# chao1224/MoleculeSDE

Hardware: AMD Instinct MI355X
Metric: molecules/sec pretrain step (SchNet+SDE VE, bs256) (higher is better)
Workload: dtype f32; 1 GPU; PCQM4Mv2-shaped pretrain step: GIN5x300 + SchNet(6x128f,51g,rc10) + EBM_node_dot_prod contrastive + SDEModel2Dto3D_02 VE; fwd+bwd+Adam; molecules_per_gpu=256, global_batch=256, parallelism=dp1

## Files before the change

### include/msde_hip.h

```cpp
#ifndef MSDE_HIP_H
#define MSDE_HIP_H

#ifdef __cplusplus
extern "C" {
#endif

#define MSDE_EINVAL (-1)
#define MSDE_EUNSUP (-2)

int msde_abi_version(void);
const char* msde_target_arch(void);

int msde_radius_count(const float* pos, const int* batch, const int* mol_ptr, int N, float r2,
                      int max_nbr, int* deg, void* stream);
int msde_exclusive_scan_i32(const int* in, int* out, int n, void* stream);
int msde_radius_fill(const float* pos, const int* batch, const int* mol_ptr, int N, float r2,
                     int max_nbr, const int* rowptr, int* src, int* dst, float* dist, int E_cap,
                     void* stream);


int msde_plan_build(const int* x_raw, int K, const int* atom_off, const int* bond_src, const int* bond_dst,
                    const int* bond_attr, const int* bond_off, const int* mol_atoms, const int* mol_bonds,
                    int B, int N_cap, int Eb_cap, int Ee_cap, int P_cap, int Er_cap, int max_nbr, int* mol_ptr,
                    int* bond_ptr, int* pair_ptr, int* sizes, int* batch_i32, int* atom_codes, int* z_codes, int* b_rowptr,
// ... 419 lines not shown
                              const unsigned long long* group_seed, const int* group_ptr, int G, int n, int max_group_atoms,
                              float snr, float scale_eps, float* x, float* x_mean, void* stream);
int msde_pc_predictor_grouped(const float* out, const float* pos, const float* noise, const float* par, const long long* step,
                              const unsigned long long* group_seed, const int* group_ptr, int G, int n, float* x, float* x_mean,
                              int* group_bad, void* stream);
int msde_l1_energy_force_loss(const float* E, const float* y, int B, const float* dE, const float* f, int n3, float fsign, float ce,
                              float cf, float* loss, float* gE, float* gdE, void* stream);
int msde_randperm(int n, int count, unsigned long long seed, const unsigned long long* seed_dev, int* out,
                  const int* rows_dev, void* stream);
int msde_ve_perturb(const float* pos, const float* noise, const long long* draws, const int* batch, int N,
                    int B, int T, float eps, float sigma_min, float sigma_max, float* pos_out,
                    float* std_out, void* stream);
int msde_ve_perturb_rng(const float* pos, const int* batch, int N, int B, int T, float eps, float sigma_min,
                        float sigma_max, unsigned long long seed, const unsigned long long* seed_dev,
                        float* noise_out, float* pos_out, float* std_out, void* stream);
int msde_ve_pos_loss_fwd(const float* scores, const float* noise, const float* std, float anneal_power,
                         const int* mol_ptr, int N, int B, float* mol_ws, float* loss, void* stream);
int msde_ve_pos_loss_bwd(const float* scores, const float* noise, const float* std, float anneal_power,
                         const int* mol_ptr, const int* batch, int N, int B, const float* g_loss,
                         float* g_scores, void* stream);

int msde_gat_tail_blocks(int N);
int msde_gat_tail_fwd(const float* x, const float* res, const float* ln1_g, const float* ln1_b,
                      const float* W0, const float* b0, const float* W3, const float* b3,
                      const float* ln2_g, const float* ln2_b, int N, int D, float eps1, float eps2,
                      float p_drop, unsigned long long seed, const unsigned long long* seed_dev,
                      int silu_out, float* out, float* y1, float* h0, float* x2, void* stream);
int msde_gat_tail_bwd(const float* g_out, const float* x, const float* y1, const float* h0,
                      const float* x2, const float* ln1_g, const float* W0, const float* W3,
                      const float* ln2_g, const float* ln2_b, int N, int D, float eps1, float eps2,
                      float p_drop, unsigned long long seed, const unsigned long long* seed_dev,
                      int silu_out, float* g_x, float* g_res, float* g_x2, float* a, float* g_h0,
                      float* ln_part, const int* rows_dev, void* stream);

long long msde_escore_mol_saved_floats(int N);
int msde_escore_mol_fwd(const void* const* params, const float* x0, const float* edge_attr, int ld_ea,
                        const float* basis, const int* mol_ptr, int B, const int* rowptr, const int* src,
                        const int* dst, int N, int E, int hidden, int heads, int hidden_coff, int n_max, float p_att,
                        float p_ffn, unsigned long long seed0, const unsigned long long* seed_dev, float eps1,
                        float eps2, float* out, float* saved, void* stream);

long long msde_escore_mol_score_scratch_floats(int E);
int msde_escore_mol_score(const void* const* params, const float* x0, const float* pos, const float* edge_2D, int ld_e2d,
                          int has_dist, const int* mol_ptr, int B, const int* rowptr, const int* src, const int* dst, int N, int E,
                          int hidden, int heads, int hidden_coff, int n_max, float eps1, float eps2, float* scratch, float* out,
                          void* stream);

long long msde_escore_mol_slab_floats(void);
int msde_escore_mol_bwd(const void* const* params, const float* x0, const float* edge_attr, int ld_ea,
                        const float* basis, const int* mol_ptr, int B, const int* rowptr, const int* src,
                        const int* dst, const int* rowptr_s, const int* perm_s, int N, int E, int hidden, int heads,
                        int hidden_coff, int n_max, float p_att, float p_ffn, unsigned long long seed0,
                        const unsigned long long* seed_dev, float eps1, float eps2, const float* saved,
                        const float* g_out, float* g_x0, float* g_edge_attr, int ld_gea, float* slabs, void* stream);

int msde_molnet_head_fwd(const float* h, int ldh, int M, int D, const int* mol_ptr, int B, const int* row_bound,
                         const float* W, const float* bias, int T, float* pool, float* logits, void* stream);
int msde_molnet_bce(const float* logits, const float* y, int B, int T, double* loss_mat, double* stats, float* dlogits,
                    void* stream);
int msde_molnet_head_bwd(const float* dlogits, int B, int T, const float* W, int D, const int* mol_ptr,
                         const int* row_bound, int M, float* dh, int ldh, void* stream);

int msde_qm9_head_train(const float* out, int ldo, int B, int D, const float* W, const float* b, const float* y, int ldy,
                        float mean, float std, int mode, float* pred, float* loss, float* dout, float* dW, float* db,
                        double* loss_acc, void* stream);
int msde_qm9_head_eval(const float* out, int ldo, int B, int D, const float* W, const float* b, const float* y, int ldy,
// ... 26 lines not shown
```

### moleculesde_amd/_lib.py

```python
import ctypes
import os

_HERE = os.path.dirname(os.path.abspath(__file__))
LIB_PATH = os.path.join(_HERE, "csrc", "libmsde_hip.so")

P = ctypes.c_void_p
I = ctypes.c_int
F = ctypes.c_float
LL = ctypes.c_longlong
ULL = ctypes.c_ulonglong

SIGNATURES = {
    "msde_abi_version": [],
    "msde_target_arch": [],
    "msde_radius_count": [P, P, P, I, F, I, P, P],
    "msde_exclusive_scan_i32": [P, P, I, P],
    "msde_radius_fill": [P, P, P, I, F, I, P, P, P, P, I, P],
    "msde_segment_sum_rows": [P, I, P, P, I, I, F, P, I, P],
    "msde_segment_sum_rows2": [P, I, P, P, P, P, I, I, F, P, I, P],
    "msde_pair_gather_add": [P, P, I, P, P, I, I, P, P],
    "msde_pair_gather_add_stats": [P, P, I, P, P, I, I, P, P, P, P],
    "msde_segment_sum_rows_bn": [P, P, I, P, P, I, I, P, P, P, P, I, P],
    "msde_pair_strip": [],
    "msde_pair_bn_dgrad_stats": [P, I, P, P, P, P, P, I, I, I, P, P, P, P],
# ... 119 lines not shown
    "msde_res_layernorm_bwd": [P, P, P, P, P, I, I, P, P, P, P, P],
    "msde_bn_fwd": [P, I, I, P, P, F, F, P, P, I, P, P, P, P, P, P],
    "msde_bn_bwd": [P, P, P, P, P, P, I, I, I, P, P, P, P, P, P],
    "msde_adam_flat": [P, P, P, P, LL, P, P, P, I, F, F, F, F, F, P],
    "msde_ssp_fwd": [P, LL, P, P],
    "msde_ssp_bwd": [P, P, LL, P, P],
    "msde_silu_dropout_fwd": [P, LL, F, ULL, P, P, P],
    "msde_silu_dropout_bwd": [P, P, LL, F, ULL, P, P, P],
    "msde_dropout_rows_fwd": [P, I, I, P, F, ULL, I, P, P, P],
    "msde_dropout_rows_bwd": [P, I, I, P, F, ULL, I, P, P, P],
    "msde_molnet_head_fwd": [P, I, I, I, P, I, P, P, P, I, P, P, P],
    "msde_molnet_bce": [P, P, I, I, P, P, P, P],
    "msde_molnet_head_bwd": [P, I, I, P, I, P, P, I, P, I, P],
    "msde_qm9_head_train": [P, I, I, I, P, P, P, I, F, F, I, P, P, P, P, P, P, P],
    "msde_qm9_head_eval": [P, I, I, I, P, P, P, I, F, F, P, P, P],
    "msde_mul_add_fwd": [P, P, P, LL, P, P],
    "msde_mul_add_bwd": [P, P, P, LL, P, P, P],
    "msde_pc_corrector": [P, P, P, P, P, ULL, I, F, F, P, P, P],
    "msde_pc_predictor": [P, P, P, P, P, ULL, I, P, P, P],
    "msde_pc_corrector_grouped": [P, P, P, P, P, P, P, I, I, I, F, F, P, P, P],
    "msde_pc_predictor_grouped": [P, P, P, P, P, P, P, I, I, P, P, P, P],
    "msde_l1_energy_force_loss": [P, P, I, P, P, I, F, F, F, P, P, P, P],
    "msde_l1_energy_force_loss_acc": [P, P, I, P, P, I, F, F, F, P, P, P, P, P],
    "msde_md17_eval_accumulate": [P, P, I, P, P, I, P, P],
    "msde_md17_gather_batch": [P, P, P, I, I, P, P, I, I, P, P, P, P],
    "msde_randperm": [I, I, ULL, P, P, P, P],
    "msde_ve_perturb": [P, P, P, P, I, I, I, F, F, F, P, P, P],
    "msde_ve_perturb_rng": [P, P, I, I, I, F, F, F, ULL, P, P, P, P, P],
    "msde_ve_pos_loss_fwd": [P, P, P, F, P, I, I, P, P, P],
    "msde_ve_pos_loss_bwd": [P, P, P, F, P, P, I, I, P, P, P],
    "msde_gat_tail_blocks": [I],
    "msde_gat_tail_fwd": [P, P, P, P, P, P, P, P, P, P, I, I, F, F, F, ULL, P, I, P, P, P, P, P],
    "msde_gat_tail_bwd": [P, P, P, P, P, P, P, P, P, P, I, I, F, F, F, ULL, P, I, P, P, P, P, P, P, P, P],
    "msde_escore_mol_saved_floats": [I],
    "msde_escore_mol_fwd": [P, P, P, I, P, P, I, P, P, P, I, I, I, I, I, I, F, F, ULL, P, F, F, P, P, P],
    "msde_escore_mol_score": [P, P, P, P, I, I, P, I, P, P, P, I, I, I, I, I, I, F, F, P, P, P],
    "msde_escore_mol_score_scratch_floats": [I],
    "msde_escore_mol_slab_floats": [],
    "msde_escore_mol_bwd": [P, P, P, I, P, P, I, P, P, P, P, P, I, I, I, I, I, I, F, F, ULL, P, F, F, P, P, P, P, I, P, P],
    "msde_chunk_elems": [],
    "msde_gather_chunks": [P, I, P, P],
    "msde_adam_chunks": [P, P, I, P, P, P, P, P, I, F, F, F, F, F, P],
}


class GemmDesc(ctypes.Structure):
    _fields_ = [("A", P), ("A2", P), ("B", P), ("B2", P), ("bias", P), ("bias2", P), ("C", P), ("Z", P), ("R", P),
                ("rowscale", P),
                ("a_gs", LL), ("b_gs", LL), ("bias_gs", LL), ("c_gs", LL), ("r_gs", LL), ("b_kblk_stride", LL),
                ("M", I), ("N", I), ("K1", I), ("K2", I),
                ("lda", I), ("lda2", I), ("ldb", I), ("ldb2", I), ("ldc", I), ("ldz", I), ("ldr", I),
                ("act", I), ("act_lo", I), ("act_hi", I), ("epi", I), ("flags", I), ("groups", I),
                ("b_kblk_log2", I), ("alpha", F)]


class RsDesc(ctypes.Structure):
    _fields_ = [("A", P), ("A2", P), ("B", P), ("bias", P), ("C", P), ("Z", P), ("R", P), ("Res", P), ("A_out", P),
                ("xf0", P), ("xf1", P), ("xf2", P), ("xf3", P), ("xf4", P), ("stats", P), ("stats_z", P),
                ("stats_mean", P), ("m_valid", P),
                ("M", I), ("N", I), ("K", I),
                ("lda", I), ("lda2", I), ("ldb", I), ("ldc", I), ("ldz", I), ("ldr", I), ("ldres", I), ("lda_out", I),
                ("ld_sz", I),
                ("act", I), ("epi", I), ("flags", I), ("axf", I), ("stats_mode", I), ("rt", I), ("splits", I)]


RS_AXF_NONE, RS_AXF_AFFINE, RS_AXF_BNBWD, RS_AXF_RELU, RS_VEC_STORE = 0, 1, 2, 4, 8
# ... 64 lines not shown
```

### moleculesde_amd/build.py

```python
import os
import subprocess
import sys
from concurrent.futures import ThreadPoolExecutor

HERE = os.path.dirname(os.path.abspath(__file__))
CSRC = os.path.join(HERE, "csrc")
OBJ = os.path.join(CSRC, "build")
LIB = os.path.join(CSRC, "libmsde_hip.so")
SOURCES = ["graph.hip", "gin.hip", "schnet.hip", "cfconv_fused.hip", "cfconv_fused_bwd.hip", "cfconv_pair.hip",
           "sde2d3d.hip", "linear.hip", "gemm_ex.hip", "gemm_rs.hip", "gemm_t2.hip", "gemm_t2_a1.hip", "gemm_t2_a2.hip", "dense_head.hip", "dense_pc.hip", "plan.hip", "dd.hip", "norm.hip",
           "contrastive.hip", "contrastive_infonce.hip", "optim.hip", "pointwise.hip", "gat_tail.hip", "escore_mol.hip", "escore_mol_bwd.hip",
           "molnet_head.hip", "qm9_head.hip", "md17.hip"]
HEADERS = [os.path.join(CSRC, "msde_common.h"), os.path.join(CSRC, "gemm_rs.h"), os.path.join(CSRC, "gemm_rs_epi.h"), os.path.join(CSRC, "gemm_t2.h"), os.path.join(CSRC, "escore_mol.h"),
           os.path.join(HERE, "..", "include", "msde_hip.h")]


def _flags():
    return ["--offload-arch=gfx950", "-O3", "-std=c++17", "-fPIC", "-Wno-unused-result", "-Wno-unused-value"] + \
        os.environ.get("MSDE_HIPCC_FLAGS", "").split()


def _stale(target, deps):
    if not os.path.exists(target):
        return True
    t = os.path.getmtime(target)
    return any(os.path.exists(d) and os.path.getmtime(d) > t for d in deps)


def needs_build():
    srcs = [os.path.join(CSRC, s) for s in SOURCES if os.path.exists(os.path.join(CSRC, s))]
    return _stale(LIB, srcs + HEADERS)


def build(force=False, verbose=True):
    if not force and not needs_build():
        return LIB
    hipcc = os.environ.get("HIPCC", "/opt/rocm/bin/hipcc")
    os.makedirs(OBJ, exist_ok=True)
    flags = _flags()
    stamp = os.path.join(OBJ, "flags.txt")
    old = open(stamp).read() if os.path.exists(stamp) else None
    if old != " ".join(flags):
        force = True
    jobs, objs = [], []
    for s in SOURCES:
        src = os.path.join(CSRC, s)
# ... 25 lines not shown
```

### moleculesde_amd/csrc/gat_tail.hip

```cpp
#include "msde_common.h"

#define GT_THREADS 256
#ifndef GT_LPR
#define GT_LPR 8
#endif
#define GT_ROWS (GT_THREADS / GT_LPR)

__device__ __forceinline__ float gt_sigmoid(float x) {
  float e = expf(-fabsf(x));
  float r = 1.f / (1.f + e);
  return x >= 0.f ? r : e * r;
}

template <int C>
__device__ __forceinline__ float gt_row_sum(float s) {
  s += __shfl_xor(s, 1);
  s += __shfl_xor(s, 2);
  if (GT_LPR >= 8) s += __shfl_xor(s, 4);
  if (GT_LPR >= 16) s += __shfl_xor(s, 8);
  return s;
}
template <int C>
__device__ __forceinline__ void gt_layernorm(const float (&v)[C], float eps, float& mu, float& rs) {
  constexpr float invD = 1.f / (float)(C * GT_LPR);
  float s = 0.f;
#pragma unroll
  for (int k = 0; k < C; ++k) s += v[k];
  mu = gt_row_sum<C>(s) * invD;
  float q = 0.f;
#pragma unroll
  for (int k = 0; k < C; ++k) q = fmaf(v[k] - mu, v[k] - mu, q);
  rs = rsqrtf(gt_row_sum<C>(q) * invD + eps);
}
// ... 171 lines not shown
    float m = 1.f;
    if (p_drop > 0.f) m = msde_uniform(seed, (unsigned long long)(off + j)) >= p_drop ? scale : 0.f;
    t2[j] = a * m;
    u[j] = u[j] * m * da;
  }
  if (live) { gt_store<C>(a_o, off, t2); gt_store<C>(g_h0_o, off, u); }
  gt_gather<C>(u, full);
  gt_matvec_t<C>(W0s, q, full, g);
  if (live) gt_store<C>(g_res, off, g);
  gt_load<C>(x, off, u);
  gt_layernorm<C>(u, eps1, mu, rs);
  c1 = 0.f; c2 = 0.f;
#pragma unroll
  for (int k = 0; k < C; ++k) {
    u[k] = (u[k] - mu) * rs;
    red[rowl][2 * D + q * C + k] = lv * g[k] * u[k];
    red[rowl][3 * D + q * C + k] = lv * g[k];
    float gg = g[k] * prm[q * C + k];
    c1 += gg; c2 = fmaf(gg, u[k], c2);
  }
  c1 = gt_row_sum<C>(c1) * (1.f / D); c2 = gt_row_sum<C>(c2) * (1.f / D);
#pragma unroll
  for (int k = 0; k < C; ++k) t2[k] = rs * (g[k] * prm[q * C + k] - c1 - u[k] * c2);
  if (live) gt_store<C>(g_x, off, t2);
  __syncthreads();
  for (int t = threadIdx.x; t < 4 * D; t += GT_THREADS) {
    float acc = 0.f;
#pragma unroll 8
    for (int r = 0; r < GT_ROWS; ++r) acc += red[r][t];
    ln_part[(size_t)blockIdx.x * 4 * D + t] = acc;
  }
}

extern "C" int msde_gat_tail_blocks(int N) { return (N + GT_ROWS - 1) / GT_ROWS; }

extern "C" int msde_gat_tail_fwd(const float* x, const float* res, const float* ln1_g, const float* ln1_b, const float* W0,
                                 const float* b0, const float* W3, const float* b3, const float* ln2_g,
                                 const float* ln2_b, int N, int D, float eps1, float eps2, float p_drop,
                                 unsigned long long seed, const unsigned long long* seed_dev, int silu_out, float* out,
                                 float* y1, float* h0, float* x2, void* stream) {
  if (N < 0 || !x || !res || !ln1_g || !ln1_b || !W0 || !b0 || !W3 || !b3 || !ln2_g || !ln2_b || !out || !y1 || !h0 || !x2)
    return MSDE_EINVAL;
  if (p_drop < 0.f || p_drop >= 1.f) return MSDE_EINVAL;
  if (D != 32) return MSDE_EUNSUP;
  if (N == 0) return 0;
  MSDE_LAUNCH(gat_tail_fwd_kernel<32>, dim3(msde_gat_tail_blocks(N)), dim3(GT_THREADS), 0, as_stream(stream), x, res, ln1_g,
              ln1_b, W0, b0, W3, b3, ln2_g, ln2_b, N, eps1, eps2, p_drop, seed, seed_dev, silu_out, out, y1, h0, x2);
  MSDE_CHECK_LAUNCH();
  return 0;
}

extern "C" int msde_gat_tail_bwd(const float* g_out, const float* x, const float* y1, const float* h0, const float* x2,
                                 const float* ln1_g, const float* W0, const float* W3, const float* ln2_g,
                                 const float* ln2_b, int N, int D, float eps1, float eps2, float p_drop,
                                 unsigned long long seed, const unsigned long long* seed_dev, int silu_out, float* g_x,
                                 float* g_res, float* g_x2, float* a, float* g_h0, float* ln_part, const int* rows_dev,
                                 void* stream) {
  if (N < 0 || !g_out || !x || !y1 || !h0 || !x2 || !ln1_g || !W0 || !W3 || !ln2_g || !ln2_b || !g_x || !g_res || !g_x2 ||
      !a || !g_h0 || !ln_part)
    return MSDE_EINVAL;
  if (p_drop < 0.f || p_drop >= 1.f) return MSDE_EINVAL;
  if (D != 32) return MSDE_EUNSUP;
  if (N == 0) return 0;
  MSDE_LAUNCH(gat_tail_bwd_kernel<32>, dim3(msde_gat_tail_blocks(N)), dim3(GT_THREADS), 0, as_stream(stream), g_out, x, y1,
              h0, x2, ln1_g, W0, W3, ln2_g, ln2_b, N, rows_dev, eps1, eps2, p_drop, seed, seed_dev, silu_out, g_x, g_res, g_x2,
              a, g_h0,
              ln_part);
  MSDE_CHECK_LAUNCH();
  return 0;
}
```

### moleculesde_amd/csrc/graph.hip

```cpp
#include "msde_common.h"

__global__ void radius_count_kernel(const float* __restrict__ pos, const int* __restrict__ batch,
                                    const int* __restrict__ mol_ptr, int N, float r2, int max_nbr,
                                    int* __restrict__ deg) {
  int i = blockIdx.x * blockDim.x + threadIdx.x;
  if (i >= N) return;
  int m = batch[i];
  int j0 = mol_ptr[m], j1 = mol_ptr[m + 1];
  float xi = pos[3 * i], yi = pos[3 * i + 1], zi = pos[3 * i + 2];
  int cnt = 0;
  for (int j = j0; j < j1 && cnt < max_nbr; ++j) {
    if (j == i) continue;
    float dx = xi - pos[3 * j], dy = yi - pos[3 * j + 1], dz = zi - pos[3 * j + 2];
    float d2 = dx * dx + dy * dy + dz * dz;
    cnt += (d2 < r2) ? 1 : 0;
  }
  deg[i] = cnt;
}

__global__ void radius_fill_kernel(const float* __restrict__ pos, const int* __restrict__ batch,
                                   const int* __restrict__ mol_ptr, int N, float r2, int max_nbr,
                                   const int* __restrict__ rowptr, int* __restrict__ src,
                                   int* __restrict__ dst, float* __restrict__ dist, int E_cap) {
  int i = blockIdx.x * blockDim.x + threadIdx.x;
  if (i < N) {
    int m = batch[i];
    int j0 = mol_ptr[m], j1 = mol_ptr[m + 1];
    float xi = pos[3 * i], yi = pos[3 * i + 1], zi = pos[3 * i + 2];
    int slot = rowptr[i];
    int cnt = 0;
    for (int j = j0; j < j1 && cnt < max_nbr; ++j) {
      if (j == i) continue;
      float dx = xi - pos[3 * j], dy = yi - pos[3 * j + 1], dz = zi - pos[3 * j + 2];
// ... 195 lines not shown
  if (mean != 0.f) scale = 1.f / (float)max(s1 - s0, 1);
  const T* R = reinterpret_cast<const T*>(rows);
  T* O = reinterpret_cast<T*>(out);
  for (int c = lane; c < cols; c += tpr) {
    T acc = vzero<V>();
    int s = s0 + el;
    for (; s + 3 * epl < s1; s += 4 * epl) {
      int e0 = perm ? perm[s] : s, e1 = perm ? perm[s + epl] : s + epl;
      int e2 = perm ? perm[s + 2 * epl] : s + 2 * epl, e3 = perm ? perm[s + 3 * epl] : s + 3 * epl;
      T v0 = R[(size_t)e0 * ldi_cols + c], v1 = R[(size_t)e1 * ldi_cols + c];
      T v2 = R[(size_t)e2 * ldi_cols + c], v3 = R[(size_t)e3 * ldi_cols + c];
      acc = vadd(vadd(vadd(vadd(acc, v0), v1), v2), v3);
    }
    for (; s < s1; s += epl) {
      int e = perm ? perm[s] : s;
      acc = vadd(acc, R[(size_t)e * ldi_cols + c]);
    }
    if (rowptr2 != nullptr && live) {
      const int q1 = rowptr2[i + 1];
      for (int q = rowptr2[i] + el; q < q1; q += epl) {
        int e = perm2 ? perm2[q] : q;
        acc = vadd(acc, R[(size_t)e * ldi_cols + c]);
      }
    }
    for (int o = tpr; o < group; o <<= 1) {
      float* a = reinterpret_cast<float*>(&acc);
#pragma unroll
      for (int k = 0; k < V; ++k) a[k] += __shfl_xor(a[k], o);
    }
    if (live && el == 0) O[(size_t)i * ldo_cols + c] = vscale(acc, scale);
  }
}

static inline int seg_epl(int N, int tpr) {
  const int force = 0;
  if (force) return force * tpr <= 64 ? force : 1;
  const int wide = 0;
  if (tpr >= 32 && !wide) return 1;
  int epl = 1;
  while (epl < 4 && tpr * epl * 2 <= 64 && (long)N * tpr * epl < 256L * 1024) epl *= 2;
  return epl;
}

extern "C" int msde_segment_sum_rows2(const float* rows, int ldi, const int* rowptr, const int* perm, const int* rowptr2,
                                      const int* perm2, int N, int D, float scale_by_inv_count, float* out, int ldo,
                                      void* stream) {
  if (N < 0 || D <= 0 || !rowptr || !out) return MSDE_EINVAL;
  if (ldo <= 0) ldo = D;
  if (ldi <= 0) ldi = D;
  if (ldo < D || ldi < D) return MSDE_EINVAL;
  if (N == 0) return 0;
  const bool vec = D % 4 == 0 && ldo % 4 == 0 && ldi % 4 == 0 &&
                   ((reinterpret_cast<uintptr_t>(rows) | reinterpret_cast<uintptr_t>(out)) & 15) == 0;
  if (vec) {
    int cols = D / 4, tpr = pick_tpr(cols), epl = seg_epl(N, tpr), rpb = 256 / (tpr * epl);
    MSDE_LAUNCH(segment_sum_rows_kernel<4>, dim3((N + rpb - 1) / rpb), dim3(256), 0, as_stream(stream), rows,
                       rowptr, perm, rowptr2, perm2, N, cols, ldi / 4, tpr, epl, scale_by_inv_count, out, ldo / 4);
  } else {
    int cols = D, tpr = pick_tpr(cols), epl = seg_epl(N, tpr), rpb = 256 / (tpr * epl);
    MSDE_LAUNCH(segment_sum_rows_kernel<1>, dim3((N + rpb - 1) / rpb), dim3(256), 0, as_stream(stream), rows,
                       rowptr, perm, rowptr2, perm2, N, cols, ldi, tpr, epl, scale_by_inv_count, out, ldo);
  }
  MSDE_CHECK_LAUNCH();
  return 0;
}

extern "C" int msde_segment_sum_rows(const float* rows, int ldi, const int* rowptr, const int* perm, int N, int D,
                                     float scale_by_inv_count, float* out, int ldo, void* stream) {
  return msde_segment_sum_rows2(rows, ldi, rowptr, perm, nullptr, nullptr, N, D, scale_by_inv_count, out, ldo, stream);
}

template <int V>
__global__ void pair_gather_add_kernel(const float* __restrict__ A, const float* __restrict__ B,
                                       const int* __restrict__ src, const int* __restrict__ dst, int E, int cols,
                                       int ld_cols, int tpr, float* __restrict__ out) {
  using T = typename VecT<V>::type;
// ... 557 lines not shown
```

### moleculesde_amd/geom3d/sde_2d_to_3d.py

```python
import torch
import torch.nn as nn
import torch.nn.functional as F

from .. import dd as _dd, escore as _escore, hip, plan as _plan, wcache
from . import nn as _nn
from .sde import VESDE, VPSDE

EPSILON = 1e-6
import os as _os
FUSE_GAT_TAIL = True
NOISE_IN_KERNEL = True
FUSE_FRAME = True
STATIC_FEATURE_CACHE = True
FUSE_HEAD_MIX = True
FUSE_EDGE_EMB = True
MOL_KERNEL = True
MOL_KERNEL_SCORE = True
MOL_KERNEL_TRAIN = False
FANOUT_EDGE_ATTR = True
FUSE_PAIR_LINEAR = True


class GaussianFourierProjection(nn.Module):

    def __init__(self, embedding_size, scale=1.0):
        super().__init__()
        self.W = nn.Parameter(torch.randn(embedding_size) * scale, requires_grad=False)


class TransformerConv(nn.Module):

    def __init__(self, in_channels, out_channels, heads, dropout, edge_dim):
        super().__init__()
        self.heads, self.out_channels, self.dropout = heads, out_channels, dropout
        self.lin_key = _nn.Linear(in_channels, heads * out_channels)
        self.lin_query = _nn.Linear(in_channels, heads * out_channels)
        self.lin_value = _nn.Linear(in_channels, heads * out_channels)
        self.lin_edge = _nn.Linear(edge_dim, heads * out_channels, bias=False)
        self.lin_skip = _nn.Linear(in_channels, heads * out_channels, bias=True)

    def fusion_sets(self):
        return [[self.lin_query.weight, self.lin_key.weight, self.lin_value.weight, self.lin_skip.weight],
                [self.lin_query.bias, self.lin_key.bias, self.lin_value.bias, self.lin_skip.bias]]

    def forward(self, x, edge_attr, plan, seed, seed_dev=None, ee_all=None, col=0, shared=None):
        Ws, bs = self.fusion_sets()
        W, b = hip.cat_params(Ws), hip.cat_params(bs)
        x_res, qkvs = _nn.linear_fork(x, W, b)
        p = self.dropout if self.training else 0.0
        if ee_all is not None:
            return x_res, hip.edge_attention_fused(qkvs, ee_all, plan, self.heads, p, seed, seed_dev, col, shared)
        ee = self.lin_edge(edge_attr)
        return x_res, hip.edge_attention_fused(qkvs, ee, plan, self.heads, p, seed, seed_dev)


class GATLayer(nn.Module):
    def __init__(self, n_head, hidden_dim, dropout=0.2):
        super().__init__()
        assert hidden_dim % n_head == 0
        self.MHA = TransformerConv(hidden_dim, hidden_dim // n_head, n_head, dropout, hidden_dim)
        self.FFN = nn.Sequential(_nn.Linear(hidden_dim, hidden_dim), nn.SiLU(), nn.Dropout(dropout),
                                 _nn.Linear(hidden_dim, hidden_dim))
        self.norm1 = nn.LayerNorm(hidden_dim)
        self.norm2 = nn.LayerNorm(hidden_dim)

    def forward(self, plan, node_attr, edge_attr, seed, seed_dev=None, ee_all=None, col=0, shared=None, silu_out=False):
        node_attr, x = self.MHA(node_attr, edge_attr, plan, seed, seed_dev, ee_all, col, shared)
        p = self.FFN[2].p if self.training else 0.0
        if x.size(-1) == 32 and FUSE_GAT_TAIL:
            return hip.gat_tail(x, node_attr, self.norm1, self.FFN[0], self.FFN[3], self.norm2, p, seed ^ 0x46464E,
                                seed_dev, silu_out)
        if x.size(-1) % 4 == 0:
            node_attr = hip.res_layernorm(x, node_attr, self.norm1.weight, self.norm1.bias, self.norm1.eps)
            node_attr, f0 = self.FFN[0].fork(node_attr)
            x = self.FFN[3](hip.silu_dropout(f0, p, seed ^ 0x46464E, seed_dev))
            out = hip.res_layernorm(x, node_attr, self.norm2.weight, self.norm2.bias, self.norm2.eps)
            return hip.silu_dropout(out) if silu_out else out
        node_attr = node_attr + self.norm1(x)
        x = self.FFN(node_attr)
        out = node_attr + self.norm2(x)
        return F.silu(out) if silu_out else out


class _EquiLayer(nn.Module):

    def __init__(self):
# ... 274 lines not shown
```

### moleculesde_amd/hip.py

```python
import ctypes

import weakref as _weakref

import torch

from . import _lib


from ._torchabi import _stream, _p, _f32, _i32


import contextlib as _contextlib

_BOUNDS = {}


@_contextlib.contextmanager
def row_bounds(bounds):
    global _BOUNDS
    for t in bounds.values():
        assert t.dtype == torch.int32 and t.is_cuda and t.numel() >= 1
    prev, _BOUNDS = _BOUNDS, {int(c): t for c, t in bounds.items()}
    try:
        yield
# ... 824 lines not shown
    def forward(ctx, q, k, v, ee, plan, heads, p_drop, seed, seed_dev):
        q, k, v, ee = _f32(q), _f32(k), _f32(v), _f32(ee)
        N, D = q.shape
        Ch = D // heads
        alpha = torch.empty(plan.E, heads, dtype=torch.float32, device=q.device)
        out = torch.empty_like(q)
        _lib.call("msde_edge_attention_fwd", _p(q), _p(k), _p(v), _p(None), D, _p(ee), 0, _p(plan.rowptr), _p(plan.src), N,
                  heads, Ch, float(p_drop), int(seed), _p(seed_dev), _p(alpha), _p(out), _stream())
        ctx.save_for_backward(q, k, v, ee, alpha)
        ctx.plan, ctx.heads, ctx.p_drop, ctx.seed, ctx.seed_dev = plan, heads, float(p_drop), int(seed), seed_dev
        return out

    @staticmethod
    def backward(ctx, g):
        q, k, v, ee, alpha = ctx.saved_tensors
        plan, H = ctx.plan, ctx.heads
        g = _f32(g)
        N, D = q.shape
        g_q = torch.empty_like(q)
        g_ee = torch.empty_like(ee)
        g_kpe = torch.empty_like(ee)
        g_vpe = torch.empty_like(ee)
        _lib.call("msde_edge_attention_bwd", _p(g), _p(q), _p(k), _p(v), D, _p(None), D, _p(ee), 0, _p(alpha),
                  _p(plan.rowptr), _p(plan.src), N, H, D // H, ctx.p_drop, ctx.seed, _p(ctx.seed_dev), _p(g_q), _p(g_ee),
                  _p(g_kpe), _p(g_vpe), 0, _stream())
        g_k = segment_sum_rows(g_kpe, plan.rowptr_s, plan.perm_s, N)
        g_v = segment_sum_rows(g_vpe, plan.rowptr_s, plan.perm_s, N)
        return g_q, g_k, g_v, g_ee, None, None, None, None, None


class _EdgeAttentionFused(torch.autograd.Function):

    @staticmethod
    def forward(ctx, qkvs, ee, plan, heads, p_drop, seed, seed_dev, col=0, shared=None):
        qkvs, ee = _f32(qkvs), _f32(ee)
        N, D4 = qkvs.shape
        D = D4 // 4
        Ch = D // heads
        ld_ee = ee.size(1)
        alpha = torch.empty(plan.E, heads, dtype=torch.float32, device=qkvs.device)
        out = torch.empty(N, D, dtype=torch.float32, device=qkvs.device)
        base = qkvs.data_ptr()
        pq, pk, pv, ps = (ctypes.c_void_p(base + 4 * D * j) for j in range(4))
        _lib.call("msde_edge_attention_fwd", pq, pk, pv, ps, D4, ctypes.c_void_p(ee.data_ptr() + 4 * col), ld_ee,
                  _p(plan.rowptr), _p(plan.src), N, heads, Ch, float(p_drop), int(seed), _p(seed_dev), _p(alpha), _p(out),
                  _stream())
        ctx.save_for_backward(qkvs, ee, alpha)
        ctx.plan, ctx.heads, ctx.p_drop, ctx.seed, ctx.seed_dev = plan, heads, float(p_drop), int(seed), seed_dev
        ctx.col, ctx.shared = col, shared
        if shared is not None and col == 0:
            shared.clear()
        return out

    @staticmethod
    def backward(ctx, g):
        qkvs, ee, alpha = ctx.saved_tensors
        plan, H = ctx.plan, ctx.heads
        g = _f32(g)
        N, D4 = qkvs.shape
        D = D4 // 4
        E, ld_ee = ee.shape
        g_qkvs = torch.empty_like(qkvs)
        first = True
        if ctx.shared is None or ld_ee == D:
            g_ee = torch.empty_like(ee)
        else:
            g_ee = ctx.shared.get("g_ee")
            first = g_ee is None
            if first:
                g_ee = ctx.shared["g_ee"] = torch.empty_like(ee)
                ctx.shared["left"] = ld_ee // D
            ctx.shared["left"] -= 1
            if ctx.shared["left"] == 0:
                del ctx.shared["g_ee"]
        g_kv = torch.empty(E, 2 * D, dtype=torch.float32, device=g.device)
        base, gbase = qkvs.data_ptr(), g_qkvs.data_ptr()
        pq, pk, pv = (ctypes.c_void_p(base + 4 * D * j) for j in range(3))
        gq, gk, gv, gs = (ctypes.c_void_p(gbase + 4 * D * j) for j in range(4))
        _lib.call("msde_edge_attention_bwd", _p(g), pq, pk, pv, D4, gs, D4, ctypes.c_void_p(ee.data_ptr() + 4 * ctx.col),
                  ld_ee, _p(alpha), _p(plan.rowptr), _p(plan.src), N, H, D // H, ctx.p_drop, ctx.seed, _p(ctx.seed_dev), gq,
                  ctypes.c_void_p(g_ee.data_ptr() + 4 * ctx.col), _p(g_kv), ctypes.c_void_p(g_kv.data_ptr() + 4 * D), 2 * D,
                  _stream())
        _lib.call("msde_segment_sum_rows", _p(g_kv), 0, _p(plan.rowptr_s), _p(plan.perm_s), N, 2 * D, 0.0, gk, D4, _stream())
        return g_qkvs, (g_ee if first else None), None, None, None, None, None, None, None


def edge_attention_fused(qkvs, ee, plan, heads, p_drop=0.0, seed=0, seed_dev=None, col=0, shared=None):
    return _EdgeAttentionFused.apply(qkvs, ee, plan, heads, p_drop, seed, seed_dev, col, shared)


def edge_attention(q, k, v, ee, plan, heads, p_drop=0.0, seed=0, seed_dev=None):
    return _EdgeAttention.apply(q, k, v, ee, plan, heads, p_drop, seed, seed_dev)


class _FrameMixMean(torch.autograd.Function):
    @staticmethod
    def forward(ctx, coff, basis, plan, base=None):
        coff = _f32(coff)
        base = _f32(base) if base is not None else None
        out = torch.empty(plan.N, 3, dtype=torch.float32, device=coff.device)
        _lib.call("msde_frame_mix_mean_add_fwd", _p(coff), _p(basis), _p(plan.rowptr), plan.N, _p(base), _p(out), _stream())
        ctx.save_for_backward(basis)
        ctx.plan = plan
        return out

    @staticmethod
    def backward(ctx, g):
        (basis,) = ctx.saved_tensors
        plan = ctx.plan
        g = _f32(g)
        g_coff = torch.empty(plan.E, 3, dtype=torch.float32, device=g.device)
        _lib.call("msde_frame_mix_mean_bwd", _p(g), _p(basis), _p(plan.rowptr), plan.N, plan.E, _p(g_coff), _stream())
        return g_coff, None, None, (g if ctx.needs_input_grad[3] else None)


def frame_mix_mean(coff, basis, plan, base=None):
    return _FrameMixMean.apply(coff, basis, plan, base)


class _MlpHeadMix(torch.autograd.Function):

# ... 81 lines not shown

class _GatherRowsGrad(torch.autograd.Function):

    @staticmethod
    def forward(ctx, x, idx, inv):
        ctx.save_for_backward(inv)
        return gather_rows(x, idx)

    @staticmethod
    def backward(ctx, g):
        (inv,) = ctx.saved_tensors
        return gather_rows(_f32(g), inv), None, None


def gather_rows_grad(x, idx, inv):
    return _GatherRowsGrad.apply(x, idx, inv)


def segment_reduce(x, mol_ptr, batch_i32, mean=True):
    return _SegmentMean.apply(x, mol_ptr, batch_i32, mean)


from .slabs import (_retire, EMB_BWD_SPLIT, _scratch, _ws_key, _SlabBatch, _SLABS, run_deferred_leaf_kernels, _row_stride,
                    weight_grad, weight_grad_blocks)




import os as _os

_LINEAR_MODE = "auto"


def set_linear_mode(mode):
    global _LINEAR_MODE
    assert mode in ("auto", "hip")
    _LINEAR_MODE = mode




class _PairLinear(torch.autograd.Function):

    @staticmethod
    def forward(ctx, h, W, b):
        h = _f32(h)
        M, D = h.shape
        B = weight_layout("pair_linear", (W,), (D, 2 * D), [(W, 0, 0, D, D, 0, 0, True), (W, 0, D, D, D, 0, D, True)])
        bst = weight_layout("pair_bias", (b,), (2 * D,), [(b, 0, 0, 1, D, 0, D, False)])
        AB = torch.empty(M, 2 * D, dtype=torch.float32, device=h.device)
        gemm_rs(h, B, AB, bias=bst, b_kmajor=True, N=2 * D, K=D, fallback=False)
        ctx.save_for_backward(h, W)
        ctx.deferrable = W.is_leaf and b.is_leaf
        return AB

    @staticmethod
    def backward(ctx, g):
        h, W = ctx.saved_tensors
        g = _f32(g)
        M, D = h.shape
        g1, g2 = g[:, :D], g[:, D:]
        gh = None
        if ctx.needs_input_grad[0]:
            gh = torch.empty(M, D, dtype=torch.float32, device=g.device)
            gemm_rs(g1, W, gh, b_kmajor=True, N=D, K=D, fallback=False)
            gemm_rs(g2, W[:, D:], gh, b_kmajor=True, N=D, K=D, accumulate=True, fallback=False)
# ... 657 lines not shown
        N, D = x.shape
        out, y1, h0, x2 = (torch.empty_like(x) for _ in range(4))
        seed = int(seed) & 0xFFFFFFFFFFFFFFFF
        _lib.call("msde_gat_tail_fwd", _p(x), _p(res), _p(g1), _p(b1), _p(W0), _p(b0), _p(W3), _p(b3), _p(g2), _p(b2), N, D,
                  float(eps1), float(eps2), float(p), seed, _p(seed_dev), int(silu_out), _p(out), _p(y1), _p(h0), _p(x2),
                  _stream())
        ctx.save_for_backward(x, y1, h0, x2, g1, W0, W3, g2, b2)
        ctx.cfg = (float(eps1), float(eps2), float(p), seed, seed_dev, int(silu_out))
        ctx.deferrable = all(t.is_leaf for t in (g1, b1, W0, b0, W3, b3, g2, b2))
        return out

    @staticmethod
    def backward(ctx, g):
        x, y1, h0, x2, g1, W0, W3, g2, b2 = ctx.saved_tensors
        eps1, eps2, p, seed, seed_dev, silu_out = ctx.cfg
        g = _f32(g)
        N, D = x.shape
        g_x, g_res, g_x2, a, g_h0 = (torch.empty_like(x) for _ in range(5))
        nblk = int(_lib.load().msde_gat_tail_blocks(N))
        defer = _SLABS.active and ctx.deferrable
        part = _SLABS.alloc(nblk * 4 * D, x.device) if defer else torch.empty(nblk * 4 * D, dtype=torch.float32, device=x.device)
        _lib.call("msde_gat_tail_bwd", _p(g), _p(x), _p(y1), _p(h0), _p(x2), _p(g1), _p(W0), _p(W3), _p(g2), _p(b2), N, D,
                  eps1, eps2, p, seed, _p(seed_dev), silu_out, _p(g_x), _p(g_res), _p(g_x2), _p(a), _p(g_h0), _p(part),
                  _p(bound_tensor(N)), _stream())
        ln = torch.empty(4 * D, dtype=torch.float32, device=x.device)
        if defer:
            _SLABS.add(part.data_ptr(), nblk, 4 * D, ln)
        else:
            torch.sum(part.view(nblk, 4 * D), dim=0, out=ln)
        gW3, gb3 = weight_grad(g_x2, a, True, ctx.deferrable)
        gW0, gb0 = weight_grad(g_h0, y1, True, ctx.deferrable)
        return (g_x, g_res, ln[2 * D:3 * D], ln[3 * D:], gW0, gb0, gW3, gb3, ln[:D], ln[D:2 * D],
                None, None, None, None, None, None)


def gat_tail(x, res, norm1, ffn0, ffn3, norm2, p, seed, seed_dev=None, silu_out=False):
    return _GatTail.apply(x, res, norm1.weight, norm1.bias, ffn0.weight, ffn0.bias, ffn3.weight, ffn3.bias, norm2.weight,
                          norm2.bias, norm1.eps, norm2.eps, p, seed, seed_dev, silu_out)


def chunk_elems():
    return int(_lib.load().msde_chunk_elems())


def gather_chunks(table, n_chunks, flat):
    _lib.call("msde_gather_chunks", _p(table), n_chunks, _p(flat), _stream())


def adam_chunks(p, table, n_chunks, m, v, step_dev, seg_end, seg_lr, beta1, beta2, eps, weight_decay, grad_scale=1.0):
    _lib.call("msde_adam_chunks", _p(p), _p(table), n_chunks, _p(m), _p(v), _p(step_dev), _p(seg_end), _p(seg_lr),
              int(seg_end.numel()), float(beta1), float(beta2), float(eps), float(weight_decay), float(grad_scale), _stream())


def adam_flat(p, g, m, v, step_dev, seg_end, seg_lr, beta1, beta2, eps, weight_decay, grad_scale=1.0):
    _lib.call("msde_adam_flat", _p(p), _p(g), _p(m), _p(v), p.numel(), _p(step_dev), _p(seg_end), _p(seg_lr),
              seg_lr.numel(), float(beta1), float(beta2), float(eps), float(weight_decay), float(grad_scale), _stream())


def _ld(t):
    assert t.dim() == 2 and t.dtype == torch.float32 and t.is_cuda and (t.size(1) == 1 or t.stride(1) == 1), \
        (t.shape, t.stride(), t.dtype)
    return t.stride(0) if t.size(0) > 1 else max(t.stride(0), t.size(1))


def gemm_ex(A, B, out, bias=None, A2=None, B2=None, act=None, act_cols=None, Z=None, dact_from=None, rowscale=None,
            b_kmajor=False, accumulate=False, alpha=1.0, groups=1, group_strides=None, N=None, K=None, K2=None, bias2=None,
# ... 442 lines not shown
```

Baseline: 104,700 molecules/s.

## Fuse GAT key/value segment-sum into projection backward dgrad kernel

```diff
diff --git a/include/msde_hip.h b/include/msde_hip.h
--- a/include/msde_hip.h
+++ b/include/msde_hip.h
@@ -475,6 +475,8 @@
                       float p_drop, unsigned long long seed, const unsigned long long* seed_dev,
                       int silu_out, float* g_x, float* g_res, float* g_x2, float* a, float* g_h0,
                       float* ln_part, const int* rows_dev, void* stream);
+int msde_gat_proj_bwd(const float* g_kv, const int* rowptr_s, const int* perm_s, const float* g_res,
+                      const float* W, int N, int D, float* g_qkvs, float* g_in, void* stream);
 
 long long msde_escore_mol_saved_floats(int N);
 int msde_escore_mol_fwd(const void* const* params, const float* x0, const float* edge_attr, int ld_ea,
diff --git a/moleculesde_amd/_lib.py b/moleculesde_amd/_lib.py
--- a/moleculesde_amd/_lib.py
+++ b/moleculesde_amd/_lib.py
@@ -175,6 +175,7 @@
     "msde_gat_tail_blocks": [I],
     "msde_gat_tail_fwd": [P, P, P, P, P, P, P, P, P, P, I, I, F, F, F, ULL, P, I, P, P, P, P, P],
     "msde_gat_tail_bwd": [P, P, P, P, P, P, P, P, P, P, I, I, F, F, F, ULL, P, I, P, P, P, P, P, P, P, P],
+    "msde_gat_proj_bwd": [P, P, P, P, P, I, I, P, P, P],
     "msde_escore_mol_saved_floats": [I],
     "msde_escore_mol_fwd": [P, P, P, I, P, P, I, P, P, P, I, I, I, I, I, I, F, F, ULL, P, F, F, P, P, P],
     "msde_escore_mol_score": [P, P, P, P, I, I, P, I, P, P, P, I, I, I, I, I, I, F, F, P, P, P],
diff --git a/moleculesde_amd/build.py b/moleculesde_amd/build.py
--- a/moleculesde_amd/build.py
+++ b/moleculesde_amd/build.py
@@ -11,7 +11,7 @@
            "sde2d3d.hip", "linear.hip", "gemm_ex.hip", "gemm_rs.hip", "gemm_t2.hip", "gemm_t2_a1.hip", "gemm_t2_a2.hip", "dense_head.hip", "dense_pc.hip", "plan.hip", "dd.hip", "norm.hip",
            "contrastive.hip", "contrastive_infonce.hip", "optim.hip", "pointwise.hip", "gat_tail.hip", "escore_mol.hip", "escore_mol_bwd.hip",
            "molnet_head.hip", "qm9_head.hip", "md17.hip"]
-HEADERS = [os.path.join(CSRC, "msde_common.h"), os.path.join(CSRC, "gemm_rs.h"), os.path.join(CSRC, "gemm_rs_epi.h"), os.path.join(CSRC, "gemm_t2.h"), os.path.join(CSRC, "escore_mol.h"),
+HEADERS = [os.path.join(CSRC, "msde_common.h"), os.path.join(CSRC, "gemm_rs.h"), os.path.join(CSRC, "gemm_rs_epi.h"), os.path.join(CSRC, "gemm_t2.h"), os.path.join(CSRC, "escore_mol.h"), os.path.join(CSRC, "seg_sum.h"),
            os.path.join(HERE, "..", "include", "msde_hip.h")]
 
 
diff --git a/moleculesde_amd/csrc/gat_tail.hip b/moleculesde_amd/csrc/gat_tail.hip
--- a/moleculesde_amd/csrc/gat_tail.hip
+++ b/moleculesde_amd/csrc/gat_tail.hip
@@ -1,4 +1,5 @@
 #include "msde_common.h"
+#include "seg_sum.h"
 
 #define GT_THREADS 256
 #ifndef GT_LPR
@@ -236,6 +237,97 @@
   }
 }
 
+#define GP_THREADS 128
+#define GP_ROWS (GP_THREADS / GT_LPR)
+#define GP_BATCH 16
+template <int D, int EPL>
+__global__ void __launch_bounds__(GP_THREADS)
+gat_proj_bwd_kernel(const float* __restrict__ g_kv, const int* __restrict__ rowptr_s, const int* __restrict__ perm_s,
+                    const float* __restrict__ g_res, const float* __restrict__ W, int N, float* __restrict__ g_qkvs,
+                    float* __restrict__ g_in) {
+  constexpr int C = D / GT_LPR;
+  static_assert(C == 4 && (EPL == 1 || EPL == 2 || EPL == 4), "one float4 per lane and block");
+  __shared__ __attribute__((aligned(16))) float Ws[4 * D * D];
+  __shared__ __attribute__((aligned(16))) float rowbuf[GP_ROWS][4 * D + 4];
+  const int q = threadIdx.x & (GT_LPR - 1), rowl = threadIdx.x / GT_LPR;
+  size_t i = (size_t)blockIdx.x * GP_ROWS + rowl;
+  const bool live = i < (size_t)N;
+  if (!live) i = (size_t)N - 1;
+  int s0 = 0, s1 = 0;
+  if (live) { s0 = rowptr_s[i]; s1 = rowptr_s[i + 1]; }
+  if ((reinterpret_cast<uintptr_t>(W) & 15) == 0) {
+    for (int t = threadIdx.x; t < D * D; t += GP_THREADS)
+      reinterpret_cast<float4*>(Ws)[t] = reinterpret_cast<const float4*>(W)[t];
+  } else {
+    for (int t = threadIdx.x; t < 4 * D * D; t += GP_THREADS) Ws[t] = W[t];
+  }
+  const size_t qoff = i * (4 * D) + q * C, off = i * D + q * C;
+  float blk[4][C], o[C];
+  gt_load<C>(g_qkvs, qoff, blk[0]);
+  gt_load<C>(g_qkvs, qoff + 3 * D, blk[3]);
+  if (g_res) {
+    gt_load<C>(g_res, off, o);
+  } else {
+#pragma unroll
+    for (int k = 0; k < C; ++k) o[k] = 0.f;
+  }
+  float4 pk[EPL], pv[EPL];
+#pragma unroll
+  for (int l = 0; l < EPL; ++l) { pk[l] = make_float4(0.f, 0.f, 0.f, 0.f); pv[l] = pk[l]; }
+  static_assert(GP_BATCH % 4 == 0, "a batch holds whole rounds of the partial sums");
+  int en[GP_BATCH];
+#pragma unroll
+  for (int t = 0; t < GP_BATCH; ++t) en[t] = s0 + t < s1 ? perm_s[s0 + t] : -1;
+  for (int s = s0; s < s1; s += GP_BATCH) {
+    float4 a[GP_BATCH], b[GP_BATCH];
+#pragma unroll
+    for (int t = 0; t < GP_BATCH; ++t) {
+      a[t] = make_float4(0.f, 0.f, 0.f, 0.f); b[t] = a[t];
+      if (en[t] >= 0) {
+        const float* r = g_kv + (size_t)en[t] * (2 * D) + q * C;
+        a[t] = *reinterpret_cast<const float4*>(r); b[t] = *reinterpret_cast<const float4*>(r + D);
+      }
+    }
+#pragma unroll
+    for (int t = 0; t < GP_BATCH; ++t) en[t] = s + GP_BATCH + t < s1 ? perm_s[s + GP_BATCH + t] : -1;
+#pragma unroll
+    for (int t = 0; t < GP_BATCH; ++t) {
+      float4& k4 = pk[t % EPL];
+      float4& v4 = pv[t % EPL];
+      k4.x += a[t].x; k4.y += a[t].y; k4.z += a[t].z; k4.w += a[t].w;
+      v4.x += b[t].x; v4.y += b[t].y; v4.z += b[t].z; v4.w += b[t].w;
+    }
+  }
+  if (EPL == 4) {
+    blk[1][0] = (pk[0].x + pk[1 % EPL].x) + (pk[2 % EPL].x + pk[3 % EPL].x); blk[1][1] = (pk[0].y + pk[1 % EPL].y) + (pk[2 % EPL].y + pk[3 % EPL].y);
+    blk[1][2] = (pk[0].z + pk[1 % EPL].z) + (pk[2 % EPL].z + pk[3 % EPL].z); blk[1][3] = (pk[0].w + pk[1 % EPL].w) + (pk[2 % EPL].w + pk[3 % EPL].w);
+    blk[2][0] = (pv[0].x + pv[1 % EPL].x) + (pv[2 % EPL].x + pv[3 % EPL].x); blk[2][1] = (pv[0].y + pv[1 % EPL].y) + (pv[2 % EPL].y + pv[3 % EPL].y);
+    blk[2][2] = (pv[0].z + pv[1 % EPL].z) + (pv[2 % EPL].z + pv[3 % EPL].z); blk[2][3] = (pv[0].w + pv[1 % EPL].w) + (pv[2 % EPL].w + pv[3 % EPL].w);
+  } else if (EPL == 2) {
+    blk[1][0] = pk[0].x + pk[1 % EPL].x; blk[1][1] = pk[0].y + pk[1 % EPL].y; blk[1][2] = pk[0].z + pk[1 % EPL].z; blk[1][3] = pk[0].w + pk[1 % EPL].w;
+    blk[2][0] = pv[0].x + pv[1 % EPL].x; blk[2][1] = pv[0].y + pv[1 % EPL].y; blk[2][2] = pv[0].z + pv[1 % EPL].z; blk[2][3] = pv[0].w + pv[1 % EPL].w;
+  } else {
+    blk[1][0] = pk[0].x; blk[1][1] = pk[0].y; blk[1][2] = pk[0].z; blk[1][3] = pk[0].w;
+    blk[2][0] = pv[0].x; blk[2][1] = pv[0].y; blk[2][2] = pv[0].z; blk[2][3] = pv[0].w;
+  }
+  if (live) { gt_store<C>(g_qkvs, qoff + D, blk[1]); gt_store<C>(g_qkvs, qoff + 2 * D, blk[2]); }
+#pragma unroll
+  for (int b = 0; b < 4; ++b) gt_store<C>(rowbuf[rowl], b * D + q * C, blk[b]);
+  __syncthreads();
+#pragma unroll 8
+  for (int j = 0; j < 4 * D; j += 4) {
+    const float4 g4 = *reinterpret_cast<const float4*>(&rowbuf[rowl][j]);
+    const float gj[4] = {g4.x, g4.y, g4.z, g4.w};
+#pragma unroll
+    for (int jj = 0; jj < 4; ++jj) {
+      const float4 w = *reinterpret_cast<const float4*>(Ws + (j + jj) * D + q * C);
+      o[0] = fmaf(w.x, gj[jj], o[0]); o[1] = fmaf(w.y, gj[jj], o[1]);
+      o[2] = fmaf(w.z, gj[jj], o[2]); o[3] = fmaf(w.w, gj[jj], o[3]);
+    }
+  }
+  if (live) gt_store<C>(g_in, off, o);
+}
+
 extern "C" int msde_gat_tail_blocks(int N) { return (N + GT_ROWS - 1) / GT_ROWS; }
 
 extern "C" int msde_gat_tail_fwd(const float* x, const float* res, const float* ln1_g, const float* ln1_b, const float* W0,
@@ -273,3 +365,18 @@
   MSDE_CHECK_LAUNCH();
   return 0;
 }
+
+extern "C" int msde_gat_proj_bwd(const float* g_kv, const int* rowptr_s, const int* perm_s, const float* g_res, const float* W,
+                                 int N, int D, float* g_qkvs, float* g_in, void* stream) {
+  if (N < 0 || !g_kv || !rowptr_s || !perm_s || !W || !g_qkvs || !g_in) return MSDE_EINVAL;
+  if (D != 32) return MSDE_EUNSUP;
+  if (N == 0) return 0;
+  const dim3 grid((N + GP_ROWS - 1) / GP_ROWS), block(GP_THREADS);
+  switch (seg_epl(N, pick_tpr(2 * 32 / 4))) {
+    case 4: MSDE_LAUNCH((gat_proj_bwd_kernel<32, 4>), grid, block, 0, as_stream(stream), g_kv, rowptr_s, perm_s, g_res, W, N, g_qkvs, g_in); break;
+    case 2: MSDE_LAUNCH((gat_proj_bwd_kernel<32, 2>), grid, block, 0, as_stream(stream), g_kv, rowptr_s, perm_s, g_res, W, N, g_qkvs, g_in); break;
+    default: MSDE_LAUNCH((gat_proj_bwd_kernel<32, 1>), grid, block, 0, as_stream(stream), g_kv, rowptr_s, perm_s, g_res, W, N, g_qkvs, g_in); break;
+  }
+  MSDE_CHECK_LAUNCH();
+  return 0;
+}
diff --git a/moleculesde_amd/csrc/graph.hip b/moleculesde_amd/csrc/graph.hip
--- a/moleculesde_amd/csrc/graph.hip
+++ b/moleculesde_amd/csrc/graph.hip
@@ -1,4 +1,5 @@
 #include "msde_common.h"
+#include "seg_sum.h"
 
 __global__ void radius_count_kernel(const float* __restrict__ pos, const int* __restrict__ batch,
                                     const int* __restrict__ mol_ptr, int N, float r2, int max_nbr,
@@ -260,16 +261,6 @@
   }
 }
 
-static inline int seg_epl(int N, int tpr) {
-  const int force = 0;
-  if (force) return force * tpr <= 64 ? force : 1;
-  const int wide = 0;
-  if (tpr >= 32 && !wide) return 1;
-  int epl = 1;
-  while (epl < 4 && tpr * epl * 2 <= 64 && (long)N * tpr * epl < 256L * 1024) epl *= 2;
-  return epl;
-}
-
 extern "C" int msde_segment_sum_rows2(const float* rows, int ldi, const int* rowptr, const int* perm, const int* rowptr2,
                                       const int* perm2, int N, int D, float scale_by_inv_count, float* out, int ldo,
                                       void* stream) {
diff --git a/moleculesde_amd/csrc/seg_sum.h b/moleculesde_amd/csrc/seg_sum.h
--- /dev/null
+++ b/moleculesde_amd/csrc/seg_sum.h
@@ -0,0 +1,11 @@
+#pragma once
+
+static inline int seg_epl(int N, int tpr) {
+  const int force = 0;
+  if (force) return force * tpr <= 64 ? force : 1;
+  const int wide = 0;
+  if (tpr >= 32 && !wide) return 1;
+  int epl = 1;
+  while (epl < 4 && tpr * epl * 2 <= 64 && (long)N * tpr * epl < 256L * 1024) epl *= 2;
+  return epl;
+}
diff --git a/moleculesde_amd/geom3d/sde_2d_to_3d.py b/moleculesde_amd/geom3d/sde_2d_to_3d.py
--- a/moleculesde_amd/geom3d/sde_2d_to_3d.py
+++ b/moleculesde_amd/geom3d/sde_2d_to_3d.py
@@ -9,6 +9,7 @@
 EPSILON = 1e-6
 import os as _os
 FUSE_GAT_TAIL = True
+FUSE_GAT_PROJ = True
 NOISE_IN_KERNEL = True
 FUSE_FRAME = True
 STATIC_FEATURE_CACHE = True
@@ -46,12 +47,18 @@
     def forward(self, x, edge_attr, plan, seed, seed_dev=None, ee_all=None, col=0, shared=None):
         Ws, bs = self.fusion_sets()
         W, b = hip.cat_params(Ws), hip.cat_params(bs)
-        x_res, qkvs = _nn.linear_fork(x, W, b)
+        fold = None
+        if (FUSE_GAT_PROJ and torch.is_grad_enabled() and x.requires_grad and x.is_cuda and x.size(-1) == 32 and plan.E > 0
+                and hip.linear_mode() == "auto"):
+            fold = {}
+            x_res, qkvs = hip.proj_fold(x, W, b, fold)
+        else:
+            x_res, qkvs = _nn.linear_fork(x, W, b)
         p = self.dropout if self.training else 0.0
         if ee_all is not None:
-            return x_res, hip.edge_attention_fused(qkvs, ee_all, plan, self.heads, p, seed, seed_dev, col, shared)
+            return x_res, hip.edge_attention_fused(qkvs, ee_all, plan, self.heads, p, seed, seed_dev, col, shared, fold)
         ee = self.lin_edge(edge_attr)
-        return x_res, hip.edge_attention_fused(qkvs, ee, plan, self.heads, p, seed, seed_dev)
+        return x_res, hip.edge_attention_fused(qkvs, ee, plan, self.heads, p, seed, seed_dev, fold=fold)
 
 
 class GATLayer(nn.Module):
diff --git a/moleculesde_amd/hip.py b/moleculesde_amd/hip.py
--- a/moleculesde_amd/hip.py
+++ b/moleculesde_amd/hip.py
@@ -880,7 +880,7 @@
 class _EdgeAttentionFused(torch.autograd.Function):
 
     @staticmethod
-    def forward(ctx, qkvs, ee, plan, heads, p_drop, seed, seed_dev, col=0, shared=None):
+    def forward(ctx, qkvs, ee, plan, heads, p_drop, seed, seed_dev, col=0, shared=None, fold=None):
         qkvs, ee = _f32(qkvs), _f32(ee)
         N, D4 = qkvs.shape
         D = D4 // 4
@@ -895,9 +895,11 @@
                   _stream())
         ctx.save_for_backward(qkvs, ee, alpha)
         ctx.plan, ctx.heads, ctx.p_drop, ctx.seed, ctx.seed_dev = plan, heads, float(p_drop), int(seed), seed_dev
-        ctx.col, ctx.shared = col, shared
+        ctx.col, ctx.shared, ctx.fold = col, shared, fold
         if shared is not None and col == 0:
             shared.clear()
+        if fold is not None:
+            fold.clear()
         return out
 
     @staticmethod
@@ -929,12 +931,16 @@
                   ld_ee, _p(alpha), _p(plan.rowptr), _p(plan.src), N, H, D // H, ctx.p_drop, ctx.seed, _p(ctx.seed_dev), gq,
                   ctypes.c_void_p(g_ee.data_ptr() + 4 * ctx.col), _p(g_kv), ctypes.c_void_p(g_kv.data_ptr() + 4 * D), 2 * D,
                   _stream())
-        _lib.call("msde_segment_sum_rows", _p(g_kv), 0, _p(plan.rowptr_s), _p(plan.perm_s), N, 2 * D, 0.0, gk, D4, _stream())
-        return g_qkvs, (g_ee if first else None), None, None, None, None, None, None, None
-
-
-def edge_attention_fused(qkvs, ee, plan, heads, p_drop=0.0, seed=0, seed_dev=None, col=0, shared=None):
-    return _EdgeAttentionFused.apply(qkvs, ee, plan, heads, p_drop, seed, seed_dev, col, shared)
+        if ctx.fold is not None:
+            ctx.fold["g_kv"], ctx.fold["plan"] = g_kv, plan
+        else:
+            _lib.call("msde_segment_sum_rows", _p(g_kv), 0, _p(plan.rowptr_s), _p(plan.perm_s), N, 2 * D, 0.0, gk, D4,
+                      _stream())
+        return g_qkvs, (g_ee if first else None), None, None, None, None, None, None, None, None
+
+
+def edge_attention_fused(qkvs, ee, plan, heads, p_drop=0.0, seed=0, seed_dev=None, col=0, shared=None, fold=None):
+    return _EdgeAttentionFused.apply(qkvs, ee, plan, heads, p_drop, seed, seed_dev, col, shared, fold)
 
 
 def edge_attention(q, k, v, ee, plan, heads, p_drop=0.0, seed=0, seed_dev=None):
@@ -1082,6 +1088,10 @@
 _LINEAR_MODE = "auto"
 
 
+def linear_mode():
+    return _LINEAR_MODE
+
+
 def set_linear_mode(mode):
     global _LINEAR_MODE
     assert mode in ("auto", "hip")
@@ -1805,6 +1815,39 @@
         gW0, gb0 = weight_grad(g_h0, y1, True, ctx.deferrable)
         return (g_x, g_res, ln[2 * D:3 * D], ln[3 * D:], gW0, gb0, gW3, gb3, ln[:D], ln[D:2 * D],
                 None, None, None, None, None, None)
+
+
+class _ProjFold(torch.autograd.Function):
+
+    @staticmethod
+    def forward(ctx, x, weight, bias, fold):
+        x2, w = _f32(x), _f32(weight)
+        qkvs = torch.empty(x2.size(0), w.size(0), dtype=torch.float32, device=x2.device)
+        if x2.size(0) > 0:
+            gemm_fwd(x2, weight, qkvs, bias=_f32(bias))
+        ctx.save_for_backward(x2, w)
+        ctx.fold = fold
+        ctx.deferrable = all(t.is_leaf or getattr(t, "_msde_leaf_like", False) for t in (weight, bias))
+        ctx.set_materialize_grads(False)
+        return x.detach(), qkvs
+
+    @staticmethod
+    def backward(ctx, g_res, g):
+        if g is None:
+            return g_res, None, None, None
+        x2, w = ctx.saved_tensors
+        M, K = x2.shape
+        g2 = _f32(g)
+        g_kv, plan = ctx.fold.pop("g_kv"), ctx.fold.pop("plan")
+        gx = torch.empty_like(x2)
+        _lib.call("msde_gat_proj_bwd", _p(g_kv), _p(plan.rowptr_s), _p(plan.perm_s), _p(_f32(g_res) if g_res is not None else None),
+                  _p(w), M, K, _p(g2), _p(gx), _stream())
+        gw, gb = weight_grad(g2, x2, True, ctx.deferrable)
+        return gx, gw, gb, None
+
+
+def proj_fold(x, weight, bias, fold):
+    return _ProjFold.apply(x, weight, bias, fold)
 
 
 def gat_tail(x, res, norm1, ffn0, ffn3, norm2, p, seed, seed_dev=None, silu_out=False):
```

Result: no change. 105,300 molecules/s, median of 6 (+0.6%).
